# zabaras/deep-turbulence

Hardware: AMD Instinct MI355X
Metric: flow-field samples/sec (fwd+log-det+bwd), 64x256x256x4; optimizer step: HipAdam (one-launch Adam, same update as torch.optim.Adam) (higher is better)
Workload: dtype f32

## Files before the change

### deep-turbulence_amd/csrc/tmg_mix16.hip

```cpp
#include "tmg_common.h"

typedef _Float16 h16x4 __attribute__((ext_vector_type(4)));

struct Mix16P {
    const float* x; int xs;
    const float* W; const float* bias;
    float* y; int ys;
    long npix; int C; int transposed;
    int ppi;
    const float* hh; int hs;
    float* r_out; float* y2_out;
    float* logdet;
    const float* r_in;
    const float* t2; int t2s;
    const float* g;
    const float* kappa;
    float* dtin2; int dts;
    float* dhh; int dhs;
};

template <int NT, int NP>
__global__ __launch_bounds__(256) void mix16_kernel(Mix16P p) {
    extern __shared__ __align__(16) unsigned char smem_raw[];
    h16x4* Wl = reinterpret_cast<h16x4*>(smem_raw);
    constexpr int CP = NT * 16;
    const int C = p.C;
    constexpr int WU = 8;
    for (int i0 = threadIdx.x; i0 < NT * 4 * CP; i0 += 256 * WU) {
        float4 wv[WU];
#pragma unroll
        for (int u = 0; u < WU; ++u) {
            const int i = i0 + u * 256;
            const int kq = i / CP, co = i - kq * CP;
// ... 160 lines not shown
                const bool ok = i < TOT && co < C && 4 * kq < C;
                v[u] = *reinterpret_cast<const float4*>(ok ? p.W + (size_t)co * C + 4 * kq : tmg_zero_page);
            }
        } else {
#pragma unroll
            for (int u = 0; u < UB; ++u) {
                const int i = i0 + u * 256;
                const int kq = i / CP, co = i - kq * CP;
                float f[4];
#pragma unroll
                for (int e = 0; e < 4; ++e) {
                    const int ci = 4 * kq + e;
                    const bool ok = i < TOT && co < C && ci < C;
                    f[e] = *(ok ? (p.transposed ? p.W + (size_t)ci * C + co : p.W + (size_t)co * C + ci) : tmg_zero_page);
                }
                v[u] = make_float4(f[0], f[1], f[2], f[3]);
            }
        }
#pragma unroll
        for (int u = 0; u < UB; ++u)
            if (i0 + u * 256 < TOT) Wl[i0 + u * 256] = v[u];
    }
    __syncthreads();
    const int lane = threadIdx.x & 63, wave = threadIdx.x >> 6;
    const int l16 = lane & 15, lq = lane >> 4;
    float4 bv[NT];
#pragma unroll
    for (int mt = 0; mt < NT; ++mt) {
        const int c = mt * 16 + 4 * lq;
        bv[mt] = (p.bias && c < C) ? *reinterpret_cast<const float4*>(p.bias + c) : make_float4(0.f, 0.f, 0.f, 0.f);
    }
    const long group = 16L * NP;
    constexpr int HT = NT / 2;
    const float hsc = AFF == 2 ? out_scale_of(p.kappa) : 1.f;
    for (long g0 = ((long)blockIdx.x * 4 + wave) * group; g0 < p.npix; g0 += (long)gridDim.x * 4 * group) {
        float4 xv[NP][NT];
        float ldsum = 0.f;
#pragma unroll
        for (int np = 0; np < NP; ++np)
#pragma unroll
            for (int ks = 0; ks < NT; ++ks) {
                const long px = g0 + np * 16 + l16;
                const int c = ks * 16 + 4 * lq;
                const float* a = (px < p.npix && c < C) ? p.x + (size_t)px * p.xs + c : tmg_zero_page;
                xv[np][ks] = *reinterpret_cast<const float4*>(a);
                if (AFF == 1 && ks >= HT) {
                    const int c2 = c - HT * 16;
                    const bool ok = px < p.npix;
                    const float* hp = ok ? p.hh + (size_t)px * p.hs + 2 * c2 : tmg_zero_page;
                    const float4 ha = *reinterpret_cast<const float4*>(hp), hb = *reinterpret_cast<const float4*>(hp + (ok ? 4 : 0));
                    const float sh[4] = {ha.x, ha.z, hb.x, hb.z}, rr[4] = {ha.y, ha.w, hb.y, hb.w};
                    const float xx[4] = {xv[np][ks].x, xv[np][ks].y, xv[np][ks].z, xv[np][ks].w};
                    float oo[4];
#pragma unroll
                    for (int e = 0; e < 4; ++e) {
                        const float sg = 2.f * rr[e] / (1.f + fabsf(rr[e]));
                        oo[e] = xx[e] * expf(-sg) - sh[e];
                        ldsum += ok ? sg : 0.f;
                    }
                    xv[np][ks] = make_float4(oo[0], oo[1], oo[2], oo[3]);
                    if (ok) {
                        *reinterpret_cast<float4*>(p.r_out + (size_t)px * (HT * 16) + c2) = make_float4(rr[0], rr[1], rr[2], rr[3]);
                        *reinterpret_cast<float4*>(p.y2_out + (size_t)px * (HT * 16) + c2) = xv[np][ks];
                    }
                }
            }
        if (AFF == 1) {
#pragma unroll
            for (int o = 32; o > 0; o >>= 1) ldsum += __shfl_xor(ldsum, o);
            if (lane == 0) atomicAdd(p.logdet + g0 / p.ppi, ldsum);
        }
#pragma unroll
        for (int np = 0; np < NP; ++np) {
            const long px = g0 + np * 16 + l16;
            f32x4 acc[NT];
#pragma unroll
            for (int mt = 0; mt < NT; ++mt) acc[mt] = (f32x4){bv[mt].x, bv[mt].y, bv[mt].z, bv[mt].w};
#pragma unroll
            for (int ks = 0; ks < NT; ++ks) {
                float4 a[NT];
#pragma unroll
                for (int mt = 0; mt < NT; ++mt) a[mt] = Wl[(ks * 4 + lq) * CP + mt * 16 + l16];
                const float4 b = xv[np][ks];
#pragma unroll
                for (int mt = 0; mt < NT; ++mt) acc[mt] = __builtin_amdgcn_mfma_f32_16x16x4f32(a[mt].x, b.x, acc[mt], 0, 0, 0);
#pragma unroll
                for (int mt = 0; mt < NT; ++mt) acc[mt] = __builtin_amdgcn_mfma_f32_16x16x4f32(a[mt].y, b.y, acc[mt], 0, 0, 0);
#pragma unroll
                for (int mt = 0; mt < NT; ++mt) acc[mt] = __builtin_amdgcn_mfma_f32_16x16x4f32(a[mt].z, b.z, acc[mt], 0, 0, 0);
#pragma unroll
                for (int mt = 0; mt < NT; ++mt) acc[mt] = __builtin_amdgcn_mfma_f32_16x16x4f32(a[mt].w, b.w, acc[mt], 0, 0, 0);
            }
#pragma unroll
            for (int mt = 0; mt < NT; ++mt) {
                const int c = mt * 16 + 4 * lq;
                if (AFF == 2 && mt >= HT) {
                    if (px < p.npix) {
                        const int c2 = c - HT * 16;
                        const float4 rq = *reinterpret_cast<const float4*>(p.r_in + (size_t)px * (HT * 16) + c2);
                        const float4 yq = *reinterpret_cast<const float4*>(p.t2 + (size_t)px * p.t2s + c2);
                        const float gb = p.g ? p.g[px / p.ppi] : 0.f;
                        const float rr[4] = {rq.x, rq.y, rq.z, rq.w}, yy[4] = {yq.x, yq.y, yq.z, yq.w};
                        float gi[4], da[4], dr[4];
#pragma unroll
                        for (int e = 0; e < 4; ++e) {
                            const float den = 1.f + fabsf(rr[e]);
                            const float sg = 2.f * rr[e] / den;
                            const float inv = expf(-sg);
                            const float go_ = acc[mt][e];
                            gi[e] = go_ * inv;
                            da[e] = -go_ * hsc;
                            dr[e] = hsc * (-2.f * go_ * (yy[e] * inv) + 2.f * gb) / (den * den);
                        }
                        *reinterpret_cast<float4*>(p.dtin2 + (size_t)px * p.dts + c2) = make_float4(gi[0], gi[1], gi[2], gi[3]);
                        float* dp = p.dhh + (size_t)px * p.dhs + 2 * c2;
                        *reinterpret_cast<float4*>(dp) = make_float4(da[0], dr[0], da[1], dr[1]);
                        *reinterpret_cast<float4*>(dp + 4) = make_float4(da[2], dr[2], da[3], dr[3]);
                    }
                } else if (px < p.npix && c < C) {
                    *reinterpret_cast<float4*>(p.y + (size_t)px * p.ys + c) = make_float4(acc[mt][0], acc[mt][1], acc[mt][2], acc[mt][3]);
                }
            }
        }
    }
}

template <int NT, int NP, int AFF = 0>
static int launch_mix32(const Mix16P& p, hipStream_t st) {
    const size_t lds = (size_t)NT * 4 * NT * 16 * sizeof(float4);
    if (lds > 64 * 1024) TMG_LDS_OPTIN((&mix32_kernel<NT, NP, AFF>));
    const long groups = (p.npix + 64L * NP - 1) / (64L * NP);
    const int grid = (int)(groups < 2048 ? (groups < 1 ? 1 : groups) : 2048);
    TmgProf prof(31, 2.0 * (double)p.npix * p.C * p.C, st);
    hipLaunchKernelGGL((mix32_kernel<NT, NP, AFF>), dim3(grid), dim3(256), lds, st, p);
    TMG_CHECK_LAUNCH();
    return 0;
}

extern "C" int tmg_mix_f32_affine_fwd(const void* x, const int64_t* x_d, const void* hh, const int64_t* hh_d, const void* W, const void* bias,
                                      void* y, const int64_t* y_d, void* r, void* y2, void* logdet, const int64_t* dims, hipStream_t st) {
    Mix16P p = {};
    p.x = static_cast<const float*>(x) + x_d[1]; p.xs = (int)x_d[0];
    p.hh = static_cast<const float*>(hh) + hh_d[1]; p.hs = (int)hh_d[0];
    p.y = static_cast<float*>(y) + y_d[1]; p.ys = (int)y_d[0];
    p.W = static_cast<const float*>(W); p.bias = static_cast<const float*>(bias);
    p.r_out = static_cast<float*>(r); p.y2_out = static_cast<float*>(y2); p.logdet = static_cast<float*>(logdet);
    p.npix = (long)dims[0]; p.C = (int)dims[1]; p.ppi = (int)dims[2]; p.transposed = 0;
    if ((p.C != 64 && p.C != 128) || p.xs % 4 || p.ys % 4 || p.hs % 4 || x_d[1] % 4 || y_d[1] % 4 || hh_d[1] % 4 || p.ppi <= 0 ||
        p.npix % p.ppi || p.ppi % (p.C == 64 ? 32 : 16))
        return -100;
    if (((((uintptr_t)p.x) | ((uintptr_t)p.hh) | ((uintptr_t)p.y) | ((uintptr_t)p.r_out) | ((uintptr_t)p.y2_out)) & 15)) return -100;
    if (p.npix <= 0) return 0;
    return p.C == 64 ? launch_mix32<4, 2, 1>(p, st) : launch_mix32<8, 1, 1>(p, st);
}

extern "C" int tmg_mix_f32_affine_bwd(const void* dy, const int64_t* dy_d, const void* W, const void* r, const void* t2, const int64_t* t2_d,
                                      const void* g, const void* kappa, void* dto1, void* dtin2, const int64_t* dtin2_d, void* dhh,
                                      const int64_t* dhh_d, const int64_t* dims, hipStream_t st) {
    Mix16P p = {};
    p.x = static_cast<const float*>(dy) + dy_d[1]; p.xs = (int)dy_d[0];
    p.W = static_cast<const float*>(W); p.bias = nullptr;
    p.npix = (long)dims[0]; p.C = (int)dims[1]; p.ppi = (int)dims[2]; p.transposed = 1;
    p.y = static_cast<float*>(dto1); p.ys = p.C / 2;
    p.r_in = static_cast<const float*>(r);
    p.t2 = static_cast<const float*>(t2) + t2_d[1]; p.t2s = (int)t2_d[0];
    p.g = static_cast<const float*>(g); p.kappa = static_cast<const float*>(kappa);
    p.dtin2 = static_cast<float*>(dtin2) + dtin2_d[1]; p.dts = (int)dtin2_d[0];
    p.dhh = static_cast<float*>(dhh) + dhh_d[1]; p.dhs = (int)dhh_d[0];
    if ((p.C != 64 && p.C != 128) || p.xs % 4 || p.t2s % 4 || p.dts % 4 || p.dhs % 4 || dy_d[1] % 4 || t2_d[1] % 4 || dtin2_d[1] % 4 ||
        dhh_d[1] % 4 || p.ppi <= 0 || p.npix % p.ppi)
        return -100;
    if (((((uintptr_t)p.x) | ((uintptr_t)p.y) | ((uintptr_t)p.r_in) | ((uintptr_t)p.t2) | ((uintptr_t)p.dtin2) | ((uintptr_t)p.dhh)) & 15)) return -100;
    if (p.npix <= 0) return 0;
    return p.C == 64 ? launch_mix32<4, 2, 2>(p, st) : launch_mix32<8, 1, 2>(p, st);
}

extern "C" int tmg_mix_f32(const void* x, const int64_t* x_d, const void* W, const void* bias, void* y, const int64_t* y_d,
                           const int64_t* dims, hipStream_t st) {
    Mix16P p;
    p.x = static_cast<const float*>(x) + x_d[1]; p.xs = (int)x_d[0];
    p.y = static_cast<float*>(y) + y_d[1]; p.ys = (int)y_d[0];
    p.W = static_cast<const float*>(W); p.bias = static_cast<const float*>(bias);
    p.npix = (long)dims[0]; p.C = (int)dims[1]; p.transposed = (int)dims[2];
    if (p.C < 4 || p.C % 4 || p.C > 128 || p.xs % 4 || p.ys % 4 || x_d[1] % 4 || y_d[1] % 4) return -1;
    if (p.npix <= 0) return 0;
    switch ((p.C + 15) / 16) {
        case 1: return launch_mix32<1, 8>(p, st);
        case 2: return launch_mix32<2, 4>(p, st);
        case 3: return launch_mix32<3, 2>(p, st);
        case 4: return launch_mix32<4, 2>(p, st);
        case 5: case 6: return launch_mix32<6, 1>(p, st);
        default: return launch_mix32<8, 1>(p, st);
    }
}
```

### deep-turbulence_amd/nn/modules/flowAffine.py

```python
import torch
import torch.nn as nn

import tmg_hip as H
import tmg_ops as ops
from nn.modules.convLSTM import ResidLSTMBlock
from nn.modules.denseBlock import NoNormDenseBlock
from nn.modules.flowUtils import Conv2dZeros


def _channels(in_features, cond_features):
    if in_features % 2 == 0:
        return in_features // 2 + cond_features, in_features
    raise NotImplementedError("odd channel counts are not on the TM-Glow path (reference flowAffine.py:43-46)")


class AffineCouplingLayer(nn.Module):

    def __init__(self, in_features, cond_features):
        super().__init__()
        in_channels, out_channels = _channels(in_features, cond_features)
        self.coupling_nn = nn.Sequential()
        self.coupling_nn.add_module('dense_block', NoNormDenseBlock(2, in_channels, growth_rate=1, drop_rate=0., bottleneck=False))
        self.coupling_nn.add_module('zero_conv', Conv2dZeros(in_channels + 2, out_channels))

    def run(self, xn, condn, reverse):
        db, zc = self.coupling_nn.dense_block, self.coupling_nn.zero_conv
        if zc.logscale_factor != 1:
            ch = xn.shape[3] // 2
            t = db.run([xn[..., :ch], condn])
            t = t[:2] + [torch.cat(t[2:], 3)]
            return ops.AffineFn.apply(zc.run(t, relu_in=True), xn, reverse)
        return ops.CouplingTailFn.apply(xn, condn, db.denselayer1.conv1.weight, db.denselayer2.conv1.weight, zc.conv.weight,
                                        zc.conv.bias, zc.scale, reverse, 0)

    def forward(self, x, cond):
        y, ld = self.run(H.nhwc(x), H.nhwc(cond), False)
        return H.nchw(y), ld

    def reverse(self, y, cond):
        x, ld = self.run(H.nhwc(y), H.nhwc(cond), True)
        return H.nchw(x), ld


class LSTMAffineCouplingLayer(nn.Module):

    def __init__(self, in_features, cond_features, rec_features):
        super().__init__()
        in_channels, out_channels = _channels(in_features, cond_features)
        self.resid_lstm = ResidLSTMBlock(in_channels, rec_features, in_channels, kernel_size=(3, 3))
        self.dense_nn = nn.Sequential()
        self.dense_nn.add_module('dense_block', NoNormDenseBlock(2, in_channels, growth_rate=1, drop_rate=0., bottleneck=False))
        self.out_conv = nn.Sequential()
        self.out_conv.add_module('zero_conv', Conv2dZeros(in_channels + 2, out_channels))

    def run(self, xn, condn, state, reverse, pad=0):
        chp = xn.shape[3] // 2
        db, zc = self.dense_nn.dense_block, self.out_conv.zero_conv
        if xn.requires_grad and torch.is_grad_enabled():
            xn, x1 = ops.LeadingChannelsFn.apply(xn, chp)
        else:
            x1 = xn[..., :chp]
        if pad == 0:
            out, h_next, c_next = self.resid_lstm.run([x1, condn], state, out_grad_premasked=True)
            y, ld = ops.CouplingTailFn.apply(xn, out, db.denselayer1.conv1.weight, db.denselayer2.conv1.weight, zc.conv.weight,
                                             zc.conv.bias, zc.scale, reverse, 1)
            return y, ld, (h_next, c_next)
        ch, dev = chp - pad, xn.device
        z = lambda *shape: torch.zeros(shape, device=dev, dtype=torch.float32)
        cell, oc = self.resid_lstm.convLSTM, self.resid_lstm.out_seq.LSTM_out_conv
        cin = oc.weight.shape[0]
        src = [cell.conv.weight, oc.weight, oc.bias, db.denselayer1.conv1.weight, db.denselayer2.conv1.weight, zc.conv.weight, zc.conv.bias]

        def build():
            ins = lambda w, at: torch.cat([w[:, :at], z(w.shape[0], pad, 3, 3), w[:, at:]], 1)
            gw = ins(cell.conv.weight, ch)
            ow = torch.cat([ins(oc.weight, ch), z(pad, oc.weight.shape[1] + pad, 3, 3)], 0)
            ob = torch.cat([oc.bias, z(pad)])
            w1 = torch.cat([db.denselayer1.conv1.weight, z(1, pad, 3, 3)], 1)
            w2 = ins(db.denselayer2.conv1.weight, cin)
            wz = torch.cat([ins(zc.conv.weight, cin), z(2 * pad, zc.conv.weight.shape[1] + pad, 3, 3)], 0)
            bz = torch.cat([zc.conv.bias, z(2 * pad)])
            return [gw, ow, ob, w1, w2, wz, bz]

        cache = self.__dict__.get('_derived')
        if cache is None:
            cache = self.__dict__['_derived'] = ops.DerivedCache()
        gw, ow, ob, w1, w2, wz, bz = cache.get('pad', src, (int(ch), int(pad)), build, proxies=True)
        if state is None:
            h_cur, c_cur = z(*xn.shape[:3], cell.hidden_dim), None
        else:
            h_cur, c_cur = state
        h_next, c_next = ops.ConvLSTMCellFn.apply(gw, cell.conv.bias, h_cur, c_cur, x1, condn)
        out = ops.conv([x1, condn, h_next], ow, ob, relu_out=True, _grad_premasked=True)
        y, ld = ops.CouplingTailFn.apply(xn, out, w1, w2, wz, bz, zc.scale, reverse, 1)
        return y, ld, (h_next, c_next)

# ... 11 lines not shown
```

### deep-turbulence_amd/nn/modules/flowLSTMBlock.py

```python
import os

import torch
import torch.nn as nn

import tmg_hip as H
import tmg_ops as ops
from nn.modules.actNorm import ActNorm
from nn.modules.flowAffine import AffineCouplingLayer, LSTMAffineCouplingLayer
from nn.modules.flowUtils import CheckerSqueeze, Split, Squeeze
from nn.modules.glowConv import InvertibleConv1x1, InvertibleConv1x1LU


def _make_conv(in_features, train_sampling, LUdecompose):
    cls = InvertibleConv1x1LU if LUdecompose else InvertibleConv1x1
    return cls(in_features, train_sampling=train_sampling)


class _BlockBase(nn.Module):

    def _mix_params(self, reverse):
        norm = getattr(self, 'norm', None)
        if isinstance(self.conv, InvertibleConv1x1LU):
            W = self.conv.matrix(reverse)
        else:
# ... 43 lines not shown
        return y, (ld if extra is None else ld + extra)

    def forward(self, x, cond):
        y, ld = self.run(H.nhwc(x), H.nhwc(cond), False)
        return H.nchw(y), ld

    def reverse(self, y, cond):
        x, ld = self.run(H.nhwc(y), H.nhwc(cond), True)
        return H.nchw(x), ld


class UnNormedAffineCouplingBlock(AffineCouplingBlock):

    def __init__(self, in_features, cond_features, train_sampling=True, LUdecompose=False):
        nn.Module.__init__(self)
        self.conv = _make_conv(in_features, train_sampling, LUdecompose)
        self.coupling = AffineCouplingLayer(in_features, cond_features)


class LSTMCouplingBlock(_BlockBase):

    def __init__(self, in_features, cond_features, rec_features, train_sampling=True, LUdecompose=False):
        super().__init__()
        self.norm = ActNorm(in_features)
        self.norm2 = ActNorm(in_features)
        self.conv = _make_conv(in_features, train_sampling, LUdecompose)
        self.coupling = LSTMAffineCouplingLayer(in_features, cond_features, rec_features)

    def run(self, xn, condn, state, reverse, mix=None, pad=0):
        if not isinstance(self.conv, InvertibleConv1x1LU):
            return _run_unfused(self, xn, condn, state, reverse)
        extra = self._mix_logdet(xn) if mix is None else None
        if reverse:
            t, ld, st = self.coupling.run(xn, condn, state, True, pad=pad)
            return self._mix(t, True, mix), (ld if extra is None else ld + extra), st
        y, ld, st = self.coupling.run(self._mix(xn, False, mix), condn, state, False, pad=pad)
        return y, (ld if extra is None else ld + extra), st

    def _call(self, x, cond, rec_states, reverse):
        st = None if rec_states is None else (H.nhwc(rec_states[0]), H.nhwc(rec_states[1]))
        y, ld, (h, c) = self.run(H.nhwc(x), H.nhwc(cond), st, reverse)
        return H.nchw(y), ld, (H.nchw(h), H.nchw(c))

    def forward(self, x, cond, rec_states=None):
        return self._call(x, cond, rec_states, False)

    def reverse(self, y, cond, rec_states=None):
        return self._call(y, cond, rec_states, True)


def _run_unfused(block, xn, condn, state, reverse):
    is_lstm = isinstance(block, LSTMCouplingBlock)
    norm = getattr(block, 'norm', None)
    x = H.nchw(xn)
    cond = H.nchw(condn)
    st_out = None
    if reverse:
        if is_lstm:
            st = None if state is None else (H.nchw(state[0]), H.nchw(state[1]))
            x, ld, st_out = block.coupling.reverse(x, cond, st)
        else:
            x, ld = block.coupling.reverse(x, cond)
        x, ld2 = block.conv.reverse(x)
        ld = ld + ld2
        if norm is not None:
            x, ld3 = norm.reverse(x)
# ... 269 lines not shown
```

### deep-turbulence_amd/tmg_hip.py

```python
import ctypes
import os
import weakref
import subprocess
import sys

import torch

_HERE = os.path.dirname(os.path.abspath(__file__))
LIB_PATH = os.path.join(_HERE, "libtmglow_hip.so")
CSRC = os.path.join(_HERE, "csrc")
SOURCES = ["tmg_conv.hip", "tmg_pointwise.hip", "tmg_physics.hip", "tmg_mix16.hip", "tmg_coupling.hip", "tmg_wino.hip", "tmg_thin.hip", "tmg_glue.hip", "tmg_ensemble.hip", "tmg_spectrum.hip", "tmg_scores.hip", "tmg_tspec.hip", "tmg_quant.hip", "tmg_gram.hip", "tmg_sfun.hip", "tmg_event.hip", "tmg_pdf.hip", "tmg_pod.hip", "tmg_phase.hip", "tmg_spod.hip", "tmg_budget.hip", "tmg_corr.hip", "tmg_flux.hip", "tmg_vortex.hip", "tmg_frank.hip", "tmg_xspec.hip", "tmg_lagr.hip"]
NO_PACKED_F32 = ["tmg_wino.hip", "tmg_conv.hip", "tmg_coupling.hip", "tmg_thin.hip", "tmg_mix16.hip", "tmg_spectrum.hip", "tmg_tspec.hip",
                 "tmg_pod.hip", "tmg_spod.hip", "tmg_xspec.hip"]
_lib = None

c_i64 = ctypes.c_int64
c_vp = ctypes.c_void_p

EXPORTS = [
    "tmg_conv_pack", "tmg_conv_pack_map", "tmg_conv_fwd", "tmg_conv_fwd_add", "tmg_affine_bwd_scaled", "tmg_c1_fwd_add", "tmg_conv_wgrad", "tmg_conv_wgrad_ws_floats", "tmg_conv_rep_border_fix", "tmg_conv_dgrad_direct",
    "tmg_affine_apply", "tmg_affine_apply_pass", "tmg_bn_finalize", "tmg_affine_bwd", "tmg_lstm_pointwise_fwd", "tmg_lstm_pointwise_bwd", "tmg_gauss_fwd",
    "tmg_gauss_bwd", "tmg_checker", "tmg_upsample_fwd", "tmg_upsample_bwd", "tmg_chan_reduce", "tmg_bn_bwd_apply",
    "tmg_phys_fwd", "tmg_phys_rms", "tmg_phys_bwd", "tmg_conv_wgrad_grouped", "tmg_conv_wgrad_grouped_ws_floats", "tmg_conv_pack_batched", "tmg_masked_add", "tmg_c1x2_fwd", "tmg_c1_fwd", "tmg_c1_bwd", "tmg_dense2_bwd", "tmg_dkappa", "tmg_prof_enable", "tmg_prof_collect", "tmg_mix_f16", "tmg_phys_bwd_dev", "tmg_coupling_fwd", "tmg_coupling_bwd",
    "tmg_conv_wino_pack", "tmg_conv_wino_fwd", "tmg_conv_wino_narrow", "tmg_conv_wino_wgrad", "tmg_conv_wino_wgrad_ws_floats", "tmg_mix_f32", "tmg_lu_fold_fwd", "tmg_lu_fold_bwd", "tmg_lu_fold_bwd_split", "tmg_level_finish", "tmg_conv_wgrad_thin_grouped", "tmg_mix_wgrad_grouped", "tmg_layer_planes", "tmg_conv_wino_wgrad_grouped", "tmg_conv_wino_wgrad_grouped_ws_floats", "tmg_adam_step", "tmg_chan_moments", "tmg_bn_finalize64", "tmg_mix_f32_affine_fwd", "tmg_mix_f32_affine_bwd", "tmg_conv_pack_many", "tmg_pad_halves", "tmg_coupling_fwd_halves", "tmg_coupling_bwd_halves", "tmg_fill_i64", "tmg_conv_wino_pack3", "tmg_conv_wino_fwd3", "tmg_mat_inverse", "tmg_gauss_sample", "tmg_reverse_loss_fwd", "tmg_reverse_loss_bwd", "tmg_sum_terms", "tmg_vec_sum", "tmg_level_pack", "tmg_spread2", "tmg_phys_fields", "tmg_phys_fields_bwd",
    "tmg_gauss_sample_keyed", "tmg_ens_accum", "tmg_ens_time_finalize", "tmg_ens_turb_accum", "tmg_ens_turb_finalize",
    "tmg_spec_rows", "tmg_spec_cols", "tmg_spec_accum", "tmg_spec_finalize",
    "tmg_ens_score_store", "tmg_ens_score_step",
]
PLAN_EXPORTS = ["tmg_conv_fwd_plan", "tmg_conv_wgrad_plan", "tmg_conv_rep_border_plan", "tmg_conv_wino_fwd_plan", "tmg_conv_wino_fwd3_plan",
                "tmg_conv_wino_narrow_plan", "tmg_conv_wino_wgrad_plan", "tmg_c1x2_fwd_plan", "tmg_c1_fwd_plan",
                "tmg_conv_wgrad_thin_grouped_plan", "tmg_mix_wgrad_grouped_plan"]
TSPEC_EXPORTS = ["tmg_tspec_store", "tmg_tspec_block", "tmg_tspec_finalize"]
QUANT_EXPORTS = ["tmg_ens_quant_step"]
GRAM_EXPORTS = ["tmg_ens_gram_plan", "tmg_ens_gram_step", "tmg_ens_gram_traj"]
SFUN_EXPORTS = ["tmg_ens_sfun_plan", "tmg_ens_sfun_step"]
EVENT_EXPORTS = ["tmg_ens_event_plan", "tmg_ens_event_count", "tmg_ens_event_step"]
PDF_EXPORTS = ["tmg_ens_pdf_plan", "tmg_ens_pdf_count"]
POD_EXPORTS = ["tmg_ens_pod_plan", "tmg_ens_pod_project"]
PHASE_EXPORTS = ["tmg_ens_phase_plan", "tmg_ens_phase_label", "tmg_ens_phase_accum"]
SPOD_EXPORTS = ["tmg_ens_spod_plan", "tmg_ens_spod_csd", "tmg_ens_spod_modes"]
LAYOUT_EXPORTS = ["tmg_layer_unplanes"]
BUDGET_EXPORTS = ["tmg_ens_budget_plan", "tmg_ens_budget_accum", "tmg_ens_budget_terms"]
CORR_EXPORTS = ["tmg_ens_corr_plan", "tmg_ens_corr_probe", "tmg_ens_corr_accum", "tmg_ens_corr_finalize"]
FLUX_EXPORTS = ["tmg_ens_flux_plan", "tmg_ens_flux_accum", "tmg_ens_flux_terms"]
LAGR_EXPORTS = ["tmg_ens_lagr_plan", "tmg_ens_lagr_advect", "tmg_ens_lagr_store", "tmg_ens_lagr_finalize"]
VORTEX_EXPORTS = ["tmg_ens_vortex_plan", "tmg_ens_vortex_classify", "tmg_ens_vortex_label", "tmg_ens_vortex_census"]
FRANK_EXPORTS = ["tmg_ens_frank_plan", "tmg_ens_frank_step"]
XSPEC_EXPORTS = ["tmg_ens_xspec_plan", "tmg_ens_xspec_prep", "tmg_ens_xspec_cols", "tmg_ens_xspec_accum"]
_P64 = ctypes.POINTER(ctypes.c_int64)
FLUX_ARGTYPES = {
    "tmg_ens_flux_plan": [_P64, _P64, _P64],
    "tmg_ens_flux_accum": [ctypes.c_void_p, _P64, ctypes.c_void_p, ctypes.c_void_p, ctypes.c_void_p, _P64, _P64, ctypes.c_void_p],
    "tmg_ens_flux_terms": [ctypes.c_void_p, ctypes.c_void_p, ctypes.POINTER(ctypes.c_void_p), ctypes.c_void_p, _P64, _P64, ctypes.c_void_p],
}
FRANK_ARGTYPES = {
    "tmg_ens_frank_plan": [_P64, _P64],
    "tmg_ens_frank_step": [ctypes.c_void_p, ctypes.c_void_p, ctypes.c_int64, ctypes.c_void_p, ctypes.c_void_p, ctypes.c_void_p, _P64,
                           ctypes.c_void_p],
}
XSPEC_ARGTYPES = {
    "tmg_ens_xspec_plan": [_P64, _P64],
    "tmg_ens_xspec_prep": [ctypes.c_void_p, _P64, ctypes.c_void_p, ctypes.c_void_p, ctypes.c_void_p, ctypes.c_void_p, ctypes.c_void_p,
                           ctypes.c_void_p, _P64, ctypes.c_void_p],
    "tmg_ens_xspec_cols": [ctypes.c_void_p, ctypes.c_void_p, ctypes.c_void_p, ctypes.c_void_p, ctypes.c_void_p, ctypes.c_void_p, _P64,
                           ctypes.POINTER(ctypes.c_float), ctypes.c_void_p],
    "tmg_ens_xspec_accum": [ctypes.c_void_p] * 10 + [_P64, ctypes.c_void_p],
}
RET_I64 = ("tmg_conv_wgrad_ws_floats", "tmg_conv_wgrad_grouped_ws_floats", "tmg_conv_wino_wgrad_ws_floats",
           "tmg_conv_wino_wgrad_grouped_ws_floats")


def build(force=False, verbose=False):
    from concurrent.futures import ThreadPoolExecutor
    inc = os.path.join(os.path.dirname(_HERE), "include")
    headers = [os.path.join(CSRC, "tmg_common.h"), os.path.join(CSRC, "tmg_symgram.h"), os.path.join(CSRC, "tmg_field.h"), os.path.join(CSRC, "tmg_dft.h"),
               os.path.join(inc, "tmglow_hip.h"), os.path.join(inc, "tmglow_hip_plan.h"),
               os.path.join(inc, "tmglow_hip_tspec.h"), os.path.join(inc, "tmglow_hip_quant.h"),
               os.path.join(inc, "tmglow_hip_gram.h"), os.path.join(inc, "tmglow_hip_sfun.h"),
               os.path.join(inc, "tmglow_hip_event.h"), os.path.join(inc, "tmglow_hip_pdf.h"), os.path.join(inc, "tmglow_hip_pod.h"),
               os.path.join(inc, "tmglow_hip_phase.h"), os.path.join(inc, "tmglow_hip_spod.h"), os.path.join(inc, "tmglow_hip_layout.h"),
               os.path.join(inc, "tmglow_hip_budget.h"), os.path.join(inc, "tmglow_hip_corr.h"), os.path.join(inc, "tmglow_hip_flux.h"),
               os.path.join(inc, "tmglow_hip_lagr.h"), os.path.join(inc, "tmglow_hip_vortex.h"),
               os.path.join(inc, "tmglow_hip_frank.h"), os.path.join(inc, "tmglow_hip_xspec.h")]
    hmt = max(os.path.getmtime(h) for h in headers)
    objdir = os.path.join(_HERE, "build")
    os.makedirs(objdir, exist_ok=True)
    hipcc = os.environ.get("HIPCC", "/opt/rocm/bin/hipcc")
    flags = ["--offload-arch=gfx950", "-O3", "-fPIC", "-std=c++17", "-Wno-unused-result", "-I", inc]
    jobs, objs, stamps = [], [], []
    for src in SOURCES:
        sp, ob = os.path.join(CSRC, src), os.path.join(objdir, src.replace(".hip", ".o"))
        objs.append(ob)
        extra = ["-Xclang", "-target-feature", "-Xclang", "-packed-fp32-ops"] if src in NO_PACKED_F32 else []
        line = " ".join(flags + extra)
        stamp = ob + ".flags"
        old = open(stamp).read() if os.path.exists(stamp) else None
        if force or old != line or not os.path.exists(ob) or os.path.getmtime(ob) < max(os.path.getmtime(sp), hmt):
            jobs.append([hipcc] + flags + extra + ["-c", sp, "-o", ob])
            stamps.append((stamp, line))
    if not jobs and os.path.exists(LIB_PATH) and all(os.path.getmtime(LIB_PATH) >= os.path.getmtime(o) for o in objs):
        return LIB_PATH

    def run(cmd):
        if verbose:
            print(" ".join(cmd), flush=True)
        r = subprocess.run(cmd, stderr=subprocess.PIPE, text=True)
        err = "\n".join(ln for ln in r.stderr.splitlines() if "'-packed-fp32-ops' is not a recognized feature" not in ln)
        if err.strip():
            print(err, file=sys.stderr, flush=True)
        if r.returncode != 0:
            raise subprocess.CalledProcessError(r.returncode, cmd)

    with ThreadPoolExecutor(max_workers=4) as ex:
        list(ex.map(run, jobs))
    for stamp, line in stamps:
        open(stamp, "w").write(line)
    run([hipcc, "--offload-arch=gfx950", "-shared", "-fPIC"] + objs + ["-o", LIB_PATH])
    return LIB_PATH


def lib():
    global _lib
    if _lib is None:
        if not os.path.exists(LIB_PATH):
            raise RuntimeError("libtmglow_hip.so is missing (%s): run `python -c 'import __graft_entry__ as g; g.build()'`. "
                               "There is no fallback path." % LIB_PATH)
        _lib = ctypes.CDLL(LIB_PATH)
        for name in EXPORTS:
            getattr(_lib, name).restype = c_i64 if name in RET_I64 else ctypes.c_int
        _lib.tmg_prof_name.restype = ctypes.c_char_p
        for name in PLAN_EXPORTS:
            getattr(_lib, name).restype = ctypes.c_int
            getattr(_lib, name).argtypes = PLAN_ARGTYPES[name]
        for name in TSPEC_EXPORTS + QUANT_EXPORTS + GRAM_EXPORTS + SFUN_EXPORTS + EVENT_EXPORTS + PDF_EXPORTS + POD_EXPORTS + PHASE_EXPORTS + SPOD_EXPORTS + LAYOUT_EXPORTS + BUDGET_EXPORTS + CORR_EXPORTS + LAGR_EXPORTS + VORTEX_EXPORTS:
            getattr(_lib, name).restype = ctypes.c_int
        for name in FLUX_EXPORTS:
            getattr(_lib, name).restype = ctypes.c_int
            getattr(_lib, name).argtypes = FLUX_ARGTYPES[name]
        for name in FRANK_EXPORTS:
            getattr(_lib, name).restype = ctypes.c_int
            getattr(_lib, name).argtypes = FRANK_ARGTYPES[name]
        for name in XSPEC_EXPORTS:
            getattr(_lib, name).restype = ctypes.c_int
            getattr(_lib, name).argtypes = XSPEC_ARGTYPES[name]
    return _lib


def prof_enable(on):
    lib().tmg_prof_enable(c_i64(int(on)))


def prof_kernel_id(name):
    l = lib()
    for k in range(64):
        if l.tmg_prof_name(c_i64(k)).decode() == name:
            return k
    raise KeyError(name)


def prof_collect():
    l = lib()
    nk = 64
    buf = (ctypes.c_double * (3 * nk))()
    n = l.tmg_prof_collect(buf, c_i64(nk))
    out = {}
    for k in range(n):
        if buf[3 * k] > 0:
# ... 559 lines not shown
    assert ws.numel() >= 4 * NL
    _chk(lib().tmg_level_finish(_ptr(Wz), _ptr(dWz), _ptr(Bz), _ptr(dBz), _ptr(Kp), _ptr(tmpX), _ptr(tmpC), _ptr(dW1), _ptr(dW2), _ptr(dK),
                                _ptr(ws), _i64(NL, C, ch, Cc, tmpC.shape[1] if tmpC is not None else 4), _stream()), "tmg_level_finish")


def adam_step(tab, chunks, nchunks, lr, b1, b2, eps, wd, bc1, bc2s, amsgrad):
    _chk(lib().tmg_adam_step(_ptr(tab), _ptr(chunks), _i64(nchunks, 1 if amsgrad else 0), _flts([lr, b1, b2, eps, wd, bc1, bc2s, 1.0 - b1, 1.0 - b2]), _stream()),
         "tmg_adam_step")


def mix_f32(x, W, bias, y, transposed=False):
    B, Hh, Ww, C = x.shape
    if C > 128 or C % 4:
        return False
    _chk(lib().tmg_mix_f32(_ptr(x), _d2(x), _ptr(W), _ptr(bias), _ptr(y), _d2(y), _i64(B * Hh * Ww, C, 1 if transposed else 0), _stream()),
         "tmg_mix_f32")
    return True


def mix_affine_fwd(x, hh, W, bias, y, r, y2, logdet):
    B, Hh, Ww, C = x.shape
    rc = lib().tmg_mix_f32_affine_fwd(_ptr(x), _d2(x), _ptr(hh), _d2(hh), _ptr(W), _ptr(bias), _ptr(y), _d2(y), _ptr(r), _ptr(y2),
                                      _ptr(logdet), _i64(B * Hh * Ww, C, Hh * Ww), _stream())
    return _launched(rc, "tmg_mix_f32_affine_fwd")


def mix_affine_bwd(dy, W, r, t2, g, kappa, dto1, dtin2, dhh):
    B, Hh, Ww, C = dy.shape
    rc = lib().tmg_mix_f32_affine_bwd(_ptr(dy), _d2(dy), _ptr(W), _ptr(r), _ptr(t2), _d2(t2), _ptr(g), _ptr(kappa), _ptr(dto1), _ptr(dtin2),
                                      _d2(dtin2), _ptr(dhh), _d2(dhh), _i64(B * Hh * Ww, C, Hh * Ww), _stream())
    return _launched(rc, "tmg_mix_f32_affine_bwd")


def conv_rep_border_fix(dy, w, outs, kappa=None):
    B, H, W, Cdy = dy.shape
    op, odesc, n_out = _segs(outs)
    Cx = sum(t.shape[3] for t in outs)
    _chk(lib().tmg_conv_rep_border_fix(_ptr(dy), _d2(dy), _ptr(w), _ptr(kappa), op, odesc, c_i64(n_out), _i64(B, H, W, Cdy, Cx),
                                       _stream()), "tmg_conv_rep_border_fix")


FWD_PLAN_FIELDS = ("kernel", "MT", "NTW", "WM", "WN", "TW_log2", "TH", "tiles_x", "tiles_y", "KCH", "nchunks", "grid_x", "grid_y",
                   "lds_bytes", "vec4", "ovec4")
WGRAD_PLAN_FIELDS = ("NP", "NCO", "LEAN", "ksplit", "MPIX", "TH", "TW_log2", "CITG", "PPG", "gx", "gy", "gz", "slab", "lds_bytes",
                     "ws_floats")
BORDER_PLAN_FIELDS = ("mfma", "NT", "S", "tiles", "blocks")
PLAN_ARGTYPES = {
    "tmg_conv_fwd_plan": [c_vp, c_vp, c_i64, c_vp, c_vp, c_vp, c_vp, c_vp, c_vp, c_vp, c_vp, c_vp, c_i64, c_vp, c_vp, c_vp],
    "tmg_conv_wgrad_plan": [c_vp, c_vp, c_i64, c_vp, c_vp, c_vp, c_vp, c_vp, c_vp, c_vp, c_vp, c_i64, c_vp, c_vp, c_i64, c_vp],
    "tmg_conv_rep_border_plan": [c_vp, c_vp, c_vp, c_vp, c_vp, c_vp, c_i64, c_vp, c_vp, c_vp],
    "tmg_conv_wino_fwd_plan": [c_vp, c_vp, c_i64, c_vp, c_vp, c_vp, c_vp, c_i64, c_vp, c_vp, c_vp],
    "tmg_conv_wino_fwd3_plan": [c_vp, c_vp, c_i64, c_vp, c_vp, c_vp, c_vp, c_i64, c_vp, c_vp, c_vp],
    "tmg_conv_wino_narrow_plan": [c_vp, c_vp, c_i64, c_vp, c_vp, c_vp, c_vp, c_i64, c_vp, c_vp, c_vp],
    "tmg_conv_wino_wgrad_plan": [c_vp, c_vp, c_i64, c_vp, c_vp, c_vp, c_vp, c_vp, c_i64, c_vp, c_vp, c_i64, c_vp],
    "tmg_c1x2_fwd_plan": [c_vp, c_vp, c_i64, c_vp, c_vp, c_vp, c_vp, c_vp, c_vp, c_vp, c_vp, c_vp, c_vp, c_vp],
    "tmg_c1_fwd_plan": [c_vp, c_vp, c_i64, c_vp, c_vp, c_vp, c_vp, c_vp, c_vp, c_vp, c_vp],
    "tmg_conv_wgrad_thin_grouped_plan": [c_vp, c_i64, c_vp, c_i64, c_vp, c_i64, c_vp, c_vp, c_vp, c_vp],
    "tmg_mix_wgrad_grouped_plan": [c_vp, c_i64, c_vp, c_vp, c_vp, c_vp, c_vp],
}
C1X2_PLAN_FIELDS = ("CG", "TW_log2", "TH", "tiles_x", "tiles_y", "t256", "KCH", "nchunks", "nring", "grid", "lds_bytes", "vec4")
C1_PLAN_FIELDS = ("TW_log2", "TH", "tiles_x", "tiles_y", "KCH", "nchunks", "grid", "lds_bytes", "vec4")
THIN_PLAN_FIELDS = ("SL", "CS", "TH", "dyc", "tiles_x", "tiles_y", "ntiles", "P", "xcd", "grid", "lds_bytes")
MIX_WGRAD_PLAN_FIELDS = ("CT", "U", "P", "per", "grid")
WINO_FWD_PLAN_FIELDS = ("kernel", "NPW", "Cin_pad", "nchunks", "last_groups", "ntt", "tiles_x", "tiles_y", "ntiles", "grid_x", "grid_y",
                        "max_tiles", "lds_bytes")
WINO_KERNELS = ("wino_fwd_kernel", "wino_fwdp_kernel", "wino_fwd3_kernel", "wino_nn_kernel")
# ... 1080 lines not shown
```

### deep-turbulence_amd/tmg_ops.py

```python
import collections
import math
import numbers

import os
import threading
import weakref

import torch

import tmg_hip as H

LOG5 = math.log(5.0)
LOG4 = math.log(4.0)
SPLIT_LIMITS = (-2.0, LOG5, -2.0, LOG5)
TOP_LIMITS = (0.0, 0.0, -10.0, LOG5)


class _ZeroPool:
    CHUNK = 8 << 20
    LIMIT = 2 << 20

    def __init__(self):
        self.lock = threading.Lock()
        self.cur = {}
# ... 791 lines not shown
        ctx.reverse, ctx.mode, ctx.cin = reverse, mode, cin
        ctx.save_for_backward(x, aux, D, r, y, w1, w2, wz, bz, kappa)
        return y, logdet

    @staticmethod
    def backward(ctx, dy, dld):
        x, aux, D, r, y, w1, w2, wz, bz, kappa = ctx.saved_tensors
        reverse, mode, cin = ctx.reverse, ctx.mode, ctx.cin
        dy = dy.contiguous()
        B, Hh, Ww, C = dy.shape
        ch = C // 2
        dev = dy.device
        nn_in = [x[..., :ch], aux] if mode == 0 else [aux]
        dx = empty((B, Hh, Ww, C), dev)
        dhh = empty((B, Hh, Ww, C), dev)
        g = dld.contiguous() if dld is not None else None
        H.affine_bwd(dy[..., ch:], (x if reverse else y)[..., ch:], r, g, dx[..., ch:], dhh, reverse)
        dw1, dw2, dwz, dbz, dk = carve(dev, (1, cin, 3, 3), (1, cin + 1, 3, 3), (C, cin + 2, 3, 3), (C,), kappa.shape)
        H.conv_wgrad(nn_in + [D], dhh, dwz, dbz, 3, 1, kappa=kappa, relu_in=True, pad_rep=True, cin_dst=cin + 2)
        H.dkappa(wz, dwz, bz, dbz, kappa, dk)
        G = [empty(t.shape, dev) for t in nn_in]
        GD = empty((B, Hh, Ww, 4), dev)
        wz_t = H.conv_pack(wz, 1, cin + 4)
        H.conv_fwd([dhh], wz_t, cin + 4, 3, 1, G + [GD], kappa=kappa)
        H.conv_rep_border_fix(dhh, wz_t, G + [GD], kappa=kappa)
        if mode == 0:
            H.dense2_bwd(nn_in + [D], w1, w2, dw1, dw2, GD, D, G, [dx[..., :ch], G[1]], cin, add0=dy[..., :ch], rows1=cin, rows2=cin + 1)
            daux = G[1]
        else:
            H.dense2_bwd(nn_in + [D], w1, w2, dw1, dw2, GD, D, G, [G[0]], cin, rows1=cin, rows2=cin + 1)
            H.masked_add(dx[..., :ch], src=dy[..., :ch])
            daux = G[0]
        return (dx, daux) + _defer((w1, w2, wz, bz, kappa), (dw1, dw2, dwz, dbz, dk)) + (None, None)


_MIX_PRECISION = "f16" if os.environ.get("TMG_MIX_F16") else "f32"


def set_mix_precision(kind):
    global _MIX_PRECISION
    if kind not in ("f32", "f16"):
        raise ValueError("mix precision must be 'f32' or 'f16', got %r" % (kind,))
    _MIX_PRECISION = kind


def mix_precision():
    return _MIX_PRECISION


_RECOMPUTE = [bool(os.environ.get("TMG_RECOMPUTE"))]


def set_recompute(on):
    _RECOMPUTE[0] = bool(on)


def recompute():
    return _RECOMPUTE[0]


def set_winograd_precision(kind):
    H.set_winograd_precision(kind)


def winograd_precision():
    return H.winograd_precision()
# ... 2978 lines not shown
```

Before: 1508.

## Fuse LSTM coupling tail with channel mix in reverse flow steps

Adds an autograd function that runs the LSTM-coupling affine tail and the invertible 1x1 channel mix in one fused kernel, forward and backward, for the reverse path with pad 0. It extends the mix kernel to narrow channel counts (16/32) and gives it a contiguous run-per-wave schedule that accumulates log-det per image and issues fewer atomics. The aim is to cut separate kernel launches and intermediate tensor round trips. In exchange it adds shape and alignment gates, a separate weight-gradient pass for the mix, and a fallback path.

```diff
diff --git a/deep-turbulence_amd/csrc/tmg_mix16.hip b/deep-turbulence_amd/csrc/tmg_mix16.hip
--- a/deep-turbulence_amd/csrc/tmg_mix16.hip
+++ b/deep-turbulence_amd/csrc/tmg_mix16.hip
@@ -1,4 +1,5 @@
 #include "tmg_common.h"
+#include "tmglow_hip_mixaff.h"
 
 typedef _Float16 h16x4 __attribute__((ext_vector_type(4)));
 
@@ -225,8 +226,20 @@
     }
     const long group = 16L * NP;
     constexpr int HT = NT / 2;
+    constexpr int CH = NT * 8;
+    const bool sec1 = NT > 1 || lq >= 2;
     const float hsc = AFF == 2 ? out_scale_of(p.kappa) : 1.f;
-    for (long g0 = ((long)blockIdx.x * 4 + wave) * group; g0 < p.npix; g0 += (long)gridDim.x * 4 * group) {
+    constexpr bool RUN = AFF == 1 && NT <= 2;
+    long run_begin = 0, run_end = 0;
+    if constexpr (RUN) {
+        const long G = (p.npix + group - 1) / group, per = (G + (long)gridDim.x * 4 - 1) / ((long)gridDim.x * 4);
+        run_begin = ((long)blockIdx.x * 4 + wave) * per * group;
+        run_end = run_begin + per * group < p.npix ? run_begin + per * group : p.npix;
+    }
+    float ldacc = 0.f;
+    long ldb = -1;
+    for (long g0 = RUN ? run_begin : ((long)blockIdx.x * 4 + wave) * group; g0 < (RUN ? run_end : p.npix);
+         g0 += RUN ? group : (long)gridDim.x * 4 * group) {
         float4 xv[NP][NT];
         float ldsum = 0.f;
 #pragma unroll
@@ -237,9 +250,9 @@
                 const int c = ks * 16 + 4 * lq;
                 const float* a = (px < p.npix && c < C) ? p.x + (size_t)px * p.xs + c : tmg_zero_page;
                 xv[np][ks] = *reinterpret_cast<const float4*>(a);
-                if (AFF == 1 && ks >= HT) {
-                    const int c2 = c - HT * 16;
-                    const bool ok = px < p.npix;
+                if (AFF == 1 && (NT == 1 || ks >= HT)) {
+                    const int c2 = c - CH;
+                    const bool ok = sec1 && px < p.npix;
                     const float* hp = ok ? p.hh + (size_t)px * p.hs + 2 * c2 : tmg_zero_page;
                     const float4 ha = *reinterpret_cast<const float4*>(hp), hb = *reinterpret_cast<const float4*>(hp + (ok ? 4 : 0));
                     const float sh[4] = {ha.x, ha.z, hb.x, hb.z}, rr[4] = {ha.y, ha.w, hb.y, hb.w};
@@ -251,14 +264,26 @@
                         oo[e] = xx[e] * expf(-sg) - sh[e];
                         ldsum += ok ? sg : 0.f;
                     }
-                    xv[np][ks] = make_float4(oo[0], oo[1], oo[2], oo[3]);
+                    if (sec1) xv[np][ks] = make_float4(oo[0], oo[1], oo[2], oo[3]);
                     if (ok) {
-                        *reinterpret_cast<float4*>(p.r_out + (size_t)px * (HT * 16) + c2) = make_float4(rr[0], rr[1], rr[2], rr[3]);
-                        *reinterpret_cast<float4*>(p.y2_out + (size_t)px * (HT * 16) + c2) = xv[np][ks];
+                        *reinterpret_cast<float4*>(p.r_out + (size_t)px * CH + c2) = make_float4(rr[0], rr[1], rr[2], rr[3]);
+                        *reinterpret_cast<float4*>(p.y2_out + (size_t)px * CH + c2) = xv[np][ks];
                     }
                 }
             }
-        if (AFF == 1) {
+        if constexpr (RUN) {
+            const long b = g0 / p.ppi;
+            if (b != ldb) {
+                if (ldb >= 0) {
+#pragma unroll
+                    for (int o = 32; o > 0; o >>= 1) ldacc += __shfl_xor(ldacc, o);
+                    if (lane == 0) atomicAdd(p.logdet + ldb, ldacc);
+                }
+                ldb = b;
+                ldacc = 0.f;
+            }
+            ldacc += ldsum;
+        } else if (AFF == 1) {
 #pragma unroll
             for (int o = 32; o > 0; o >>= 1) ldsum += __shfl_xor(ldsum, o);
             if (lane == 0) atomicAdd(p.logdet + g0 / p.ppi, ldsum);
@@ -287,10 +312,10 @@
 #pragma unroll
             for (int mt = 0; mt < NT; ++mt) {
                 const int c = mt * 16 + 4 * lq;
-                if (AFF == 2 && mt >= HT) {
+                if (AFF == 2 && (NT == 1 ? sec1 : mt >= HT)) {
                     if (px < p.npix) {
-                        const int c2 = c - HT * 16;
-                        const float4 rq = *reinterpret_cast<const float4*>(p.r_in + (size_t)px * (HT * 16) + c2);
+                        const int c2 = c - CH;
+                        const float4 rq = *reinterpret_cast<const float4*>(p.r_in + (size_t)px * CH + c2);
                         const float4 yq = *reinterpret_cast<const float4*>(p.t2 + (size_t)px * p.t2s + c2);
                         const float gb = p.g ? p.g[px / p.ppi] : 0.f;
                         const float rr[4] = {rq.x, rq.y, rq.z, rq.w}, yy[4] = {yq.x, yq.y, yq.z, yq.w};
@@ -316,6 +341,22 @@
             }
         }
     }
+    if constexpr (RUN) {
+        __shared__ float ld_part[4];
+        __shared__ long ld_img[4];
+#pragma unroll
+        for (int o = 32; o > 0; o >>= 1) ldacc += __shfl_xor(ldacc, o);
+        if (lane == 0) { ld_part[wave] = ldacc; ld_img[wave] = ldb; }
+        __syncthreads();
+        if (threadIdx.x == 0) {
+            for (int w = 0; w < 4; ++w) {
+                if (ld_img[w] < 0 || (w > 0 && ld_img[w] == ld_img[w - 1])) continue;
+                float sum = ld_part[w];
+                for (int v = w + 1; v < 4 && ld_img[v] == ld_img[w]; ++v) sum += ld_part[v];
+                atomicAdd(p.logdet + ld_img[w], sum);
+            }
+        }
+    }
 }
 
 template <int NT, int NP, int AFF = 0>
@@ -326,6 +367,18 @@
     const int grid = (int)(groups < 2048 ? (groups < 1 ? 1 : groups) : 2048);
     TmgProf prof(31, 2.0 * (double)p.npix * p.C * p.C, st);
     hipLaunchKernelGGL((mix32_kernel<NT, NP, AFF>), dim3(grid), dim3(256), lds, st, p);
+    TMG_CHECK_LAUNCH();
+    return 0;
+}
+
+template <int NT, int NP>
+static int launch_mix32_runs(const Mix16P& p, hipStream_t st) {
+    static_assert(NT <= 2, "mix32_kernel takes runs of groups in its narrow forward form only");
+    const size_t lds = (size_t)NT * 4 * NT * 16 * sizeof(float4);
+    const long blocks = (p.npix + 64L * NP - 1) / (64L * NP);
+    const int grid = (int)(blocks < 1024 ? (blocks < 1 ? 1 : blocks) : 1024);
+    TmgProf prof(31, 2.0 * (double)p.npix * p.C * p.C, st);
+    hipLaunchKernelGGL((mix32_kernel<NT, NP, 1>), dim3(grid), dim3(256), lds, st, p);
     TMG_CHECK_LAUNCH();
     return 0;
 }
@@ -368,6 +421,51 @@
     return p.C == 64 ? launch_mix32<4, 2, 2>(p, st) : launch_mix32<8, 1, 2>(p, st);
 }
 
+extern "C" int tmg_mix_affine_narrow_fwd(const void* x, const int64_t* x_d, const void* hh, const int64_t* hh_d, const void* W, const void* bias,
+                                         void* y, const int64_t* y_d, void* r, void* y2, void* logdet, const int64_t* dims, hipStream_t st) {
+    Mix16P p = {};
+    p.x = static_cast<const float*>(x) + x_d[1]; p.xs = (int)x_d[0];
+    p.hh = static_cast<const float*>(hh) + hh_d[1]; p.hs = (int)hh_d[0];
+    p.y = static_cast<float*>(y) + y_d[1]; p.ys = (int)y_d[0];
+    p.W = static_cast<const float*>(W); p.bias = static_cast<const float*>(bias);
+    p.r_out = static_cast<float*>(r); p.y2_out = static_cast<float*>(y2); p.logdet = static_cast<float*>(logdet);
+    p.npix = (long)dims[0]; p.C = (int)dims[1]; p.ppi = (int)dims[2]; p.transposed = 0;
+    if ((p.C != 16 && p.C != 32) || p.xs % 4 || p.ys % 4 || p.hs % 4 || x_d[1] % 4 || y_d[1] % 4 || hh_d[1] % 4 || p.xs < p.C || p.ys < p.C ||
+        p.hs < p.C || p.ppi <= 0 || p.npix % p.ppi || p.ppi % (p.C == 16 ? 64 : 32))
+        return -100;
+    if (((((uintptr_t)p.x) | ((uintptr_t)p.hh) | ((uintptr_t)p.y) | ((uintptr_t)p.r_out) | ((uintptr_t)p.y2_out)) & 15)) return -100;
+    if (p.npix <= 0) return 0;
+    return p.C == 16 ? launch_mix32_runs<1, 4>(p, st) : launch_mix32_runs<2, 2>(p, st);
+}
+
+extern "C" int tmg_mix_affine_narrow_bwd(const void* dy, const int64_t* dy_d, const void* W, const void* r, const void* t2, const int64_t* t2_d,
+                                         const void* g, const void* kappa, void* dto1, const int64_t* dto1_d, void* dtin2,
+                                         const int64_t* dtin2_d, void* dhh, const int64_t* dhh_d, const int64_t* dims, hipStream_t st) {
+    Mix16P p = {};
+    p.x = static_cast<const float*>(dy) + dy_d[1]; p.xs = (int)dy_d[0];
+    p.W = static_cast<const float*>(W); p.bias = nullptr;
+    p.npix = (long)dims[0]; p.C = (int)dims[1]; p.ppi = (int)dims[2]; p.transposed = 1;
+    p.y = static_cast<float*>(dto1) + dto1_d[1]; p.ys = (int)dto1_d[0];
+    p.r_in = static_cast<const float*>(r);
+    p.t2 = static_cast<const float*>(t2) + t2_d[1]; p.t2s = (int)t2_d[0];
+    p.g = static_cast<const float*>(g); p.kappa = static_cast<const float*>(kappa);
+    p.dtin2 = static_cast<float*>(dtin2) + dtin2_d[1]; p.dts = (int)dtin2_d[0];
+    p.dhh = static_cast<float*>(dhh) + dhh_d[1]; p.dhs = (int)dhh_d[0];
+    const int ch = p.C / 2;
+    if ((p.C != 16 && p.C != 32 && p.C != 64 && p.C != 128) || p.xs % 4 || p.ys % 4 || p.t2s % 4 || p.dts % 4 || p.dhs % 4 || dy_d[1] % 4 ||
+        dto1_d[1] % 4 || t2_d[1] % 4 || dtin2_d[1] % 4 || dhh_d[1] % 4 || p.xs < p.C || p.ys < ch || p.t2s < ch || p.dts < ch || p.dhs < p.C ||
+        p.ppi <= 0 || p.npix % p.ppi)
+        return -100;
+    if (((((uintptr_t)p.x) | ((uintptr_t)p.y) | ((uintptr_t)p.r_in) | ((uintptr_t)p.t2) | ((uintptr_t)p.dtin2) | ((uintptr_t)p.dhh)) & 15)) return -100;
+    if (p.npix <= 0) return 0;
+    switch (p.C) {
+        case 16: return launch_mix32<1, 4, 2>(p, st);
+        case 32: return launch_mix32<2, 2, 2>(p, st);
+        case 64: return launch_mix32<4, 2, 2>(p, st);
+        default: return launch_mix32<8, 1, 2>(p, st);
+    }
+}
+
 extern "C" int tmg_mix_f32(const void* x, const int64_t* x_d, const void* W, const void* bias, void* y, const int64_t* y_d,
                            const int64_t* dims, hipStream_t st) {
     Mix16P p;
diff --git a/deep-turbulence_amd/nn/modules/flowAffine.py b/deep-turbulence_amd/nn/modules/flowAffine.py
--- a/deep-turbulence_amd/nn/modules/flowAffine.py
+++ b/deep-turbulence_amd/nn/modules/flowAffine.py
@@ -53,7 +53,7 @@
         self.out_conv = nn.Sequential()
         self.out_conv.add_module('zero_conv', Conv2dZeros(in_channels + 2, out_channels))
 
-    def run(self, xn, condn, state, reverse, pad=0):
+    def run(self, xn, condn, state, reverse, pad=0, mix=None):
         chp = xn.shape[3] // 2
         db, zc = self.dense_nn.dense_block, self.out_conv.zero_conv
         if xn.requires_grad and torch.is_grad_enabled():
@@ -62,6 +62,11 @@
             x1 = xn[..., :chp]
         if pad == 0:
             out, h_next, c_next = self.resid_lstm.run([x1, condn], state, out_grad_premasked=True)
+            if mix is not None:
+                assert reverse
+                y, ld = ops.LSTMTailMixFn.apply(xn, out, mix[0], mix[1], db.denselayer1.conv1.weight, db.denselayer2.conv1.weight,
+                                                zc.conv.weight, zc.conv.bias, zc.scale)
+                return y, ld, (h_next, c_next)
             y, ld = ops.CouplingTailFn.apply(xn, out, db.denselayer1.conv1.weight, db.denselayer2.conv1.weight, zc.conv.weight,
                                              zc.conv.bias, zc.scale, reverse, 1)
             return y, ld, (h_next, c_next)
diff --git a/deep-turbulence_amd/nn/modules/flowLSTMBlock.py b/deep-turbulence_amd/nn/modules/flowLSTMBlock.py
--- a/deep-turbulence_amd/nn/modules/flowLSTMBlock.py
+++ b/deep-turbulence_amd/nn/modules/flowLSTMBlock.py
@@ -99,6 +99,12 @@
             return _run_unfused(self, xn, condn, state, reverse)
         extra = self._mix_logdet(xn) if mix is None else None
         if reverse:
+            if pad == 0:
+                Wb = self._mix_params(True) if mix is None else mix
+                if ops.lstm_tail_fusable(xn, Wb[0], Wb[1]):
+                    y, ld, st = self.coupling.run(xn, condn, state, True, mix=Wb)
+                    return y, (ld if extra is None else ld + extra), st
+                mix = Wb
             t, ld, st = self.coupling.run(xn, condn, state, True, pad=pad)
             return self._mix(t, True, mix), (ld if extra is None else ld + extra), st
         y, ld, st = self.coupling.run(self._mix(xn, False, mix), condn, state, False, pad=pad)
diff --git a/deep-turbulence_amd/tmg_hip.py b/deep-turbulence_amd/tmg_hip.py
--- a/deep-turbulence_amd/tmg_hip.py
+++ b/deep-turbulence_amd/tmg_hip.py
@@ -40,6 +40,7 @@
 PHASE_EXPORTS = ["tmg_ens_phase_plan", "tmg_ens_phase_label", "tmg_ens_phase_accum"]
 SPOD_EXPORTS = ["tmg_ens_spod_plan", "tmg_ens_spod_csd", "tmg_ens_spod_modes"]
 LAYOUT_EXPORTS = ["tmg_layer_unplanes"]
+MIXAFF_EXPORTS = ["tmg_mix_affine_narrow_fwd", "tmg_mix_affine_narrow_bwd"]
 BUDGET_EXPORTS = ["tmg_ens_budget_plan", "tmg_ens_budget_accum", "tmg_ens_budget_terms"]
 CORR_EXPORTS = ["tmg_ens_corr_plan", "tmg_ens_corr_probe", "tmg_ens_corr_accum", "tmg_ens_corr_finalize"]
 FLUX_EXPORTS = ["tmg_ens_flux_plan", "tmg_ens_flux_accum", "tmg_ens_flux_terms"]
@@ -81,7 +82,7 @@
                os.path.join(inc, "tmglow_hip_phase.h"), os.path.join(inc, "tmglow_hip_spod.h"), os.path.join(inc, "tmglow_hip_layout.h"),
                os.path.join(inc, "tmglow_hip_budget.h"), os.path.join(inc, "tmglow_hip_corr.h"), os.path.join(inc, "tmglow_hip_flux.h"),
                os.path.join(inc, "tmglow_hip_lagr.h"), os.path.join(inc, "tmglow_hip_vortex.h"),
-               os.path.join(inc, "tmglow_hip_frank.h"), os.path.join(inc, "tmglow_hip_xspec.h")]
+               os.path.join(inc, "tmglow_hip_frank.h"), os.path.join(inc, "tmglow_hip_xspec.h"), os.path.join(inc, "tmglow_hip_mixaff.h")]
     hmt = max(os.path.getmtime(h) for h in headers)
     objdir = os.path.join(_HERE, "build")
     os.makedirs(objdir, exist_ok=True)
@@ -132,7 +133,7 @@
         for name in PLAN_EXPORTS:
             getattr(_lib, name).restype = ctypes.c_int
             getattr(_lib, name).argtypes = PLAN_ARGTYPES[name]
-        for name in TSPEC_EXPORTS + QUANT_EXPORTS + GRAM_EXPORTS + SFUN_EXPORTS + EVENT_EXPORTS + PDF_EXPORTS + POD_EXPORTS + PHASE_EXPORTS + SPOD_EXPORTS + LAYOUT_EXPORTS + BUDGET_EXPORTS + CORR_EXPORTS + LAGR_EXPORTS + VORTEX_EXPORTS:
+        for name in TSPEC_EXPORTS + QUANT_EXPORTS + GRAM_EXPORTS + SFUN_EXPORTS + EVENT_EXPORTS + PDF_EXPORTS + POD_EXPORTS + PHASE_EXPORTS + SPOD_EXPORTS + LAYOUT_EXPORTS + BUDGET_EXPORTS + CORR_EXPORTS + LAGR_EXPORTS + VORTEX_EXPORTS + MIXAFF_EXPORTS:
             getattr(_lib, name).restype = ctypes.c_int
         for name in FLUX_EXPORTS:
             getattr(_lib, name).restype = ctypes.c_int
@@ -758,6 +759,23 @@
     return _launched(rc, "tmg_mix_f32_affine_bwd")
 
 
+MIX_AFFINE_GROUP = {16: 64, 32: 32, 64: 32, 128: 16}
+
+
+def mix_affine_narrow_fwd(x, hh, W, bias, y, r, y2, logdet):
+    B, Hh, Ww, C = x.shape
+    rc = lib().tmg_mix_affine_narrow_fwd(_ptr(x), _d2(x), _ptr(hh), _d2(hh), _ptr(W), _ptr(bias), _ptr(y), _d2(y), _ptr(r), _ptr(y2),
+                                         _ptr(logdet), _i64(B * Hh * Ww, C, Hh * Ww), _stream())
+    return _launched(rc, "tmg_mix_affine_narrow_fwd")
+
+
+def mix_affine_narrow_bwd(dy, W, r, t2, g, kappa, dto1, dtin2, dhh):
+    B, Hh, Ww, C = dy.shape
+    rc = lib().tmg_mix_affine_narrow_bwd(_ptr(dy), _d2(dy), _ptr(W), _ptr(r), _ptr(t2), _d2(t2), _ptr(g), _ptr(kappa), _ptr(dto1), _d2(dto1),
+                                         _ptr(dtin2), _d2(dtin2), _ptr(dhh), _d2(dhh), _i64(B * Hh * Ww, C, Hh * Ww), _stream())
+    return _launched(rc, "tmg_mix_affine_narrow_bwd")
+
+
 def conv_rep_border_fix(dy, w, outs, kappa=None):
     B, H, W, Cdy = dy.shape
     op, odesc, n_out = _segs(outs)
diff --git a/deep-turbulence_amd/tmg_ops.py b/deep-turbulence_amd/tmg_ops.py
--- a/deep-turbulence_amd/tmg_ops.py
+++ b/deep-turbulence_amd/tmg_ops.py
@@ -847,6 +847,67 @@
             H.masked_add(dx[..., :ch], src=dy[..., :ch])
             daux = G[0]
         return (dx, daux) + _defer((w1, w2, wz, bz, kappa), (dw1, dw2, dwz, dbz, dk)) + (None, None)
+
+
+def lstm_tail_envelope(C, hw):
+    group = H.MIX_AFFINE_GROUP.get(int(C))
+    return group is not None and hw > 0 and hw % group == 0
+
+
+def lstm_tail_fusable(x, Wm, bm):
+    if os.environ.get("TMG_NO_LSTM_TAIL_FUSION") is not None or _MIX_PRECISION != "f32" or not x.is_cuda or x.dtype != torch.float32:
+        return False
+    C = x.shape[3]
+    if not lstm_tail_envelope(C, x.shape[1] * x.shape[2]) or tuple(Wm.shape) != (C, C):
+        return False
+    ts = [x, Wm] + ([bm] if bm is not None else [])
+    return all(t.is_contiguous() and t.data_ptr() % 16 == 0 for t in ts)
+
+
+class LSTMTailMixFn(torch.autograd.Function):
+
+    @staticmethod
+    def forward(ctx, x, feat, Wm, bm, w1, w2, wz, bz, kappa):
+        feat = feat if feat.is_contiguous() else feat.contiguous()
+        B, Hh, Ww, C = x.shape
+        ch, cin, dev = C // 2, feat.shape[3], x.device
+        w1, w2, wz = w1.contiguous(), w2.contiguous(), wz.contiguous()
+        D = empty((B, Hh, Ww, 4), dev)
+        H.c1_fwd([feat], w1, D[..., 0:1], relu_in=True, fill4=True)
+        H.c1_fwd([feat, D], w2, D[..., 1:2], relu_in=True, w_rows=cin + 1)
+        hh = empty((B, Hh, Ww, C), dev)
+        H.conv_fwd([feat, D], H.conv_pack(wz, 0, cin + 4), C, 3, 1, [hh], bias=bz, kappa=kappa, relu_in=True, pad_rep=True)
+        out = empty((B, Hh, Ww, C), dev)
+        r, y2 = empty((B, Hh, Ww, ch), dev), empty((B, Hh, Ww, ch), dev)
+        logdet = zeros(B, dev)
+        fwd = H.mix_affine_narrow_fwd if C <= 32 else H.mix_affine_fwd
+        if not fwd(x, hh, Wm, bm, out, r, y2, logdet):
+            raise RuntimeError("LSTMTailMixFn: the fused coupling + mix launch declined a shape lstm_tail_fusable accepted: %s" % (tuple(x.shape),))
+        ctx.save_for_backward(x, feat, D, r, y2, Wm, bm, w1, w2, wz, bz, kappa)
+        return out, logdet
+
+    @staticmethod
+    def backward(ctx, dout, dld):
+        x, feat, D, r, y2, Wm, bm, w1, w2, wz, bz, kappa = ctx.saved_tensors
+        dout = dout.contiguous()
+        B, Hh, Ww, C = dout.shape
+        ch, cin, dev = C // 2, feat.shape[3], dout.device
+        dx = empty((B, Hh, Ww, C), dev)
+        dhh = empty((B, Hh, Ww, C), dev)
+        g = dld.contiguous() if dld is not None else None
+        if not H.mix_affine_narrow_bwd(dout, Wm, r, x[..., ch:], g, None, dx[..., :ch], dx[..., ch:], dhh):
+            raise RuntimeError("LSTMTailMixFn: the fused mix + coupling backward launch declined the shape %s" % (tuple(dout.shape),))
+        dWm, dbm, dw1, dw2, dwz, dbz, dk = carve(dev, (C, C), (C,), (1, cin, 3, 3), (1, cin + 1, 3, 3), (C, cin + 2, 3, 3), (C,), kappa.shape)
+        H.conv_wgrad([x[..., :ch], y2], dout, dWm.view(C, C, 1, 1), dbm, 1, 1)
+        H.conv_wgrad([feat, D], dhh, dwz, dbz, 3, 1, kappa=kappa, relu_in=True, pad_rep=True, cin_dst=cin + 2)
+        H.dkappa(wz, dwz, bz, dbz, kappa, dk)
+        G = empty(feat.shape, dev)
+        GD = empty((B, Hh, Ww, 4), dev)
+        wz_t = H.conv_pack(wz, 1, cin + 4)
+        H.conv_fwd([dhh], wz_t, cin + 4, 3, 1, [G, GD], kappa=kappa)
+        H.conv_rep_border_fix(dhh, wz_t, [G, GD], kappa=kappa)
+        H.dense2_bwd([feat, D], w1, w2, dw1, dw2, GD, D, [G], [G], cin, rows1=cin, rows2=cin + 1)
+        return (dx, G) + _defer((Wm, bm, w1, w2, wz, bz, kappa), (dWm, dbm if bm is not None else None, dw1, dw2, dwz, dbz, dk))
 
 
 _MIX_PRECISION = "f16" if os.environ.get("TMG_MIX_F16") else "f32"
diff --git a/include/tmglow_hip_mixaff.h b/include/tmglow_hip_mixaff.h
--- /dev/null
+++ b/include/tmglow_hip_mixaff.h
@@ -0,0 +1,23 @@
+#ifndef TMGLOW_HIP_MIXAFF_H
+#define TMGLOW_HIP_MIXAFF_H
+
+#include <stdint.h>
+
+#ifdef __cplusplus
+extern "C" {
+#endif
+
+struct ihipStream_t;
+
+int tmg_mix_affine_narrow_fwd(const void* x, const int64_t* x_d, const void* hh, const int64_t* hh_d, const void* W, const void* bias, void* y,
+                              const int64_t* y_d, void* r, void* y2, void* logdet, const int64_t* dims, struct ihipStream_t* st);
+
+int tmg_mix_affine_narrow_bwd(const void* dy, const int64_t* dy_d, const void* W, const void* r, const void* t2, const int64_t* t2_d,
+                              const void* g, const void* kappa, void* dto1, const int64_t* dto1_d, void* dtin2, const int64_t* dtin2_d,
+                              void* dhh, const int64_t* dhh_d, const int64_t* dims, struct ihipStream_t* st);
+
+#ifdef __cplusplus
+}
+#endif
+
+#endif
```

Measured after the change: 1501. About the same (-0.5%).
